# kuldeepbrd1/graspLDM

Measured on AMD Instinct MI355X. Metric: grasps/sec whole-node (1024-pt cloud, 100 DDIM steps), higher is better.
Workload: dtype f32 (GEMMs as split-f16 x3 partial products on the f16 matrix pipe, f32 accumulation; GroupNorm / LayerNorm / attention / scheduler in f32); 1 GPU; LDM mode, 256 synthetic 1024-pt clouds per GPU x 20 grasps, 100 DDIM steps: BASELINE.json configs[2] per GPU (configs[3] = this per-GPU workload on 8 GPUs); experiment=fpc, clouds_per_gpu=256, grasps_per_cloud=20, points=1024, ddim_steps=100, encoder=PVCNNEncoder (shipped fpc config), parallelism=cloud-sharded x1, weights=synthetic recipe seed 0, streams=3

## Files before the change

graspldm_amd/csrc/voxel_conv.hip:

```cpp
#include <hip/hip_runtime.h>
#include <stdint.h>
#include <stdio.h>
#include <stdlib.h>

#include "gldm.h"
#include "wstream.h"
#include "devstate.h"

#define GLDM_API extern "C" __attribute__((visibility("default")))

namespace {

using f32x4 = __attribute__((ext_vector_type(4))) float;
typedef __attribute__((address_space(3))) float lds_f;

#ifdef GLDM_DEBUG_KNOBS
__device__ long long g_c3_stamp[32];
#define GLDM_C3_STAMP(i) \
  do { if (blockIdx.x == 5 && blockIdx.y == (gridDim.y >> 1) && threadIdx.x == 0) g_c3_stamp[i] = (long long)__builtin_readcyclecounter(); } while (0)
#else
#define GLDM_C3_STAMP(i) do {} while (0)
#endif

template <int CTRL>
// ... 194 lines not shown
  float *s_part = lds;
#pragma unroll
  for (int mi = 0; mi < MT; ++mi) {
#pragma unroll
    for (int q = 0; q < 4; ++q) {
      const int co = 16 * mi + 4 * kq + q;
      float s = 0.f, s2 = 0.f;
#pragma unroll
      for (int ni = 0; ni < NTW; ++ni) {
        const float v = acc[mi][ni][q];
        s += v;
        s2 += v * v;
      }
      s = row16_sum(s);
      s2 = row16_sum(s2);
      if (col == 0 && co < cout) {
        s_part[(wave * MT * 16 + co) * 2] = s;
        s_part[(wave * MT * 16 + co) * 2 + 1] = s2;
      }
    }
  }
  GLDM_C3_STAMP(24);
  __syncthreads();
  GLDM_C3_STAMP(25);
  if (tid < cout) {
    float s = 0.f, s2 = 0.f;
    for (int w = 0; w < 4; ++w) {
      s += s_part[(w * MT * 16 + tid) * 2];
      s2 += s_part[(w * MT * 16 + tid) * 2 + 1];
    }
    float *p = partial + (((size_t)b * gridDim.x + blockIdx.x) * cout_total + co0 + tid) * 2;
    p[0] = s;
    p[1] = s2;
  }
  GLDM_C3_STAMP(26);
  if (out_cl) {
#pragma unroll
    for (int ni = 0; ni < NTW; ++ni)
#pragma unroll
      for (int mi = 0; mi < MT; ++mi)
        if (16 * mi + 4 * kq < cout) *reinterpret_cast<f32x4 *>(y + (size_t)gvox[ni] * cout_total + 16 * mi + 4 * kq) = acc[mi][ni];
  } else {
#pragma unroll
    for (int mi = 0; mi < MT; ++mi)
#pragma unroll
      for (int q = 0; q < 4; ++q) {
        const int co = 16 * mi + 4 * kq + q;
        if (co < cout) {
#pragma unroll
          for (int ni = 0; ni < NTW; ++ni) y[(size_t)co * r3 + gvox[ni]] = acc[mi][ni][q];
        }
      }
  }
  GLDM_C3_STAMP(21);
}

typedef __attribute__((ext_vector_type(8))) _Float16 c3_f16x8;
typedef __attribute__((ext_vector_type(2))) _Float16 c3_f16x2;
typedef __attribute__((ext_vector_type(2))) float c3_f32x2;
typedef __attribute__((ext_vector_type(4))) unsigned c3_u32x4;
constexpr int kC3Split = 2;

__device__ __forceinline__ void c3_split(const float (&x)[8], c3_u32x4 (&pl)[kC3Split]) {
#pragma unroll
  for (int q = 0; q < 4; ++q) {
    const float a = x[2 * q], b = x[2 * q + 1];
    const c3_f16x2 h = __builtin_convertvector(c3_f32x2{a, b}, c3_f16x2);
    const float ra = __builtin_fmaf((float)h[0], -1.0f, a), rb = __builtin_fmaf((float)h[1], -1.0f, b);
    pl[0][q] = __builtin_bit_cast(unsigned, h);
    pl[1][q] = __builtin_bit_cast(unsigned, __builtin_convertvector(c3_f32x2{ra, rb}, c3_f16x2));
  }
}
__device__ __forceinline__ f32x4 c3_mfma(const c3_u32x4 &a, const c3_u32x4 &b, const f32x4 &c) {
  return __builtin_amdgcn_mfma_f32_16x16x32_f16(__builtin_bit_cast(c3_f16x8, a), __builtin_bit_cast(c3_f16x8, b), c, 0, 0, 0);
}
__device__ __forceinline__ f32x4 c3_mfma3(const c3_u32x4 (&a)[kC3Split], const c3_u32x4 (&b)[kC3Split], f32x4 acc) {
  acc = c3_mfma(a[0], b[1], acc);
  acc = c3_mfma(a[1], b[0], acc);
  return c3_mfma(a[0], b[0], acc);
}

constexpr int kPairs = 14;

__device__ __forceinline__ float c3_range_pow2(float m) {
  int e = (int)((__float_as_uint(m) >> 23) & 0xffu) - 127;
  if ((e >= -8 && e < 14) || e < -100 || e > 100) return 1.0f;
  e = e < -40 ? -40 : e;
  return __uint_as_float((unsigned)(e - 13 + 127) << 23);
}
__device__ __forceinline__ float c3_pow2_inv(float s) { return __uint_as_float((254u << 23) - __float_as_uint(s)); }
__device__ __forceinline__ float c3_wave_max(float x) {
#pragma unroll
  for (int off = 32; off >= 1; off >>= 1) x = fmaxf(x, __shfl_xor(x, off, 64));
  return x;
}

template <int MT, int R, int ZB, int WAVES, bool ACT = false>
__global__ __launch_bounds__(64 * WAVES, (ZB * 16 / WAVES / 16 >= 6) ? 1 : 2) void conv3d_k3_pl_kernel(const float *__restrict__ x,
                                                                                      const float *__restrict__ wp3,
                                                                                      const float *__restrict__ bias, int cin,
                                                                                      int cout, float *__restrict__ y,
                                                                                      float *__restrict__ partial,
                                                                                      const float *__restrict__ in_coef,
                                                                                      int out_cl) {
  constexpr int r = R, NTW = ZB / WAVES, kThreads = 64 * WAVES, kZParts = R / ZB;
  constexpr int GM = MT % 3 == 0 ? 3 : (MT % 4 == 0 ? 4 : (MT % 2 == 0 ? 2 : 1));
  constexpr int GN = NTW % 3 == 0 ? 3 : (NTW % 2 == 0 ? 2 : 1);
  static_assert(R % ZB == 0 && ZB % WAVES == 0, "whole n-tiles per wave");
  constexpr int MG = MT / GM, NG = NTW / GN;
  constexpr int zp = ZB + 2, nvox = 36 * zp, r3 = r * r * r;
  constexpr int hs = (nvox + 15) & ~15;
  constexpr int kItems = 2 * nvox, kRounds = (kItems + kThreads - 1) / kThreads;
  constexpr bool kDB = R == 24 && ZB == 24;
  constexpr bool kRanged = !ACT;
  extern __shared__ float lds[];
  GLDM_C3_STAMP(0);
  __builtin_amdgcn_s_setprio(3);
  const int tid = threadIdx.x, wave = tid >> 6, lane = tid & 63;
  const int col = lane & 15, kq = lane >> 4;
  const int bpr = r / kBrick;
  const int bxy = blockIdx.x / kZParts, bz0 = (blockIdx.x % kZParts) * ZB;
  const int bx0 = (bxy / bpr) * kBrick, by0 = (bxy % bpr) * kBrick;
  const int b = blockIdx.y;
  const int cblocks = (cin + 15) >> 4, kblocks = kPairs * cblocks;
  x += (size_t)b * cin * r3;
  y += (size_t)b * cout * r3;
  const WStream wv(wp3, lane);
  typedef __attribute__((address_space(3))) c3_u32x4 lds_c4;
  constexpr int kSet = kC3Split * 2 * hs;
  lds_c4 *pl0 = (lds_c4 *)lds;

  int vb[NTW];
#pragma unroll
  for (int ni = 0; ni < NTW; ++ni) {
    const int o = 16 * (wave * NTW + ni) + col;
    const int iz = o % ZB, ixy = o / ZB, ix = ixy >> 2, iy = ixy & 3;
    vb[ni] = (ix * 6 + iy) * zp + iz + (kq & 1) * hs;
  }
  f32x4 acc[MT][NTW];
#pragma unroll
  for (int mi = 0; mi < MT; ++mi) {
    f32x4 bvv;
#pragma unroll
    for (int q = 0; q < 4; ++q) bvv[q] = bias[16 * mi + 4 * kq + q];
#pragma unroll
    for (int ni = 0; ni < NTW; ++ni) acc[mi][ni] = bvv;
  }
  int s_lds[kRounds], s_glb[kRounds];
#pragma unroll
  for (int q = 0; q < kRounds; ++q) {
    const int it = tid + q * kThreads;
    s_lds[q] = -1;
    s_glb[q] = -1;
    if (it < kItems) {
      const int h = it / nvox, v = it - h * nvox;
      const int ixy = v / zp, izp = v - ixy * zp;
      const int gx = bx0 + ixy / 6 - 1, gy = by0 + ixy % 6 - 1, gz = bz0 + izp - 1;
      s_lds[q] = h * hs + v;
      if ((unsigned)gx < (unsigned)r && (unsigned)gy < (unsigned)r && (unsigned)gz < (unsigned)r)
        s_glb[q] = (gx * r + gy) * r + gz + 8 * h * r3;
    }
  }
  {
    const c3_u32x4 z4 = c3_u32x4{0u, 0u, 0u, 0u};
#pragma unroll
    for (int q = 0; q < kRounds; ++q)
      if (s_lds[q] >= 0 && s_glb[q] < 0) {
#pragma unroll
        for (int p3 = 0; p3 < kC3Split; ++p3) {
          pl0[p3 * 2 * hs + s_lds[q]] = z4;
          if constexpr (kDB) pl0[kSet + p3 * 2 * hs + s_lds[q]] = z4;
        }
      }
  }
  float stg[kRounds][8];
  auto stage_load = [&](int cb) {
    const float *xc = x + (size_t)(cb * 16) * r3;
#pragma unroll
    for (int q = 0; q < kRounds; ++q) {
      const int g0 = s_glb[q] >= 0 ? s_glb[q] : 0;
#pragma unroll
      for (int j = 0; j < 8; ++j) stg[q][j] = xc[(size_t)j * r3 + g0];
    }
  };
  float *s_coef = lds + (kDB ? 2 : 1) * kSet * 4;
  if constexpr (ACT) {
    for (int i = tid; i < 2 * cin; i += kThreads) s_coef[i] = in_coef[(size_t)b * cin * 2 + i];
  }
  unsigned s_run_u = 0x3f800000u;
  float *rng = s_coef;
  auto stage_store = [&](int cb) {
    lds_c4 *pl = pl0 + (kDB ? (cb & 1) * kSet : 0);
#pragma unroll
    for (int q = 0; q < kRounds; ++q)
      if (s_glb[q] >= 0) {
        if constexpr (kRanged) {
          const float inv_run = __uint_as_float((254u << 23) - s_run_u);
#pragma unroll
          for (int j = 0; j < 8; ++j) stg[q][j] *= inv_run;
        }
        if constexpr (ACT) {
          const int h = (tid + q * kThreads) / nvox;
          const f32x4 *cf = reinterpret_cast<const f32x4 *>(s_coef + 2 * (16 * cb + 8 * h));
#pragma unroll
          for (int j2 = 0; j2 < 4; ++j2) {
            const f32x4 c4 = cf[j2];
            const float t0 = fmaf(stg[q][2 * j2], c4[0], c4[1]), t1 = fmaf(stg[q][2 * j2 + 1], c4[2], c4[3]);
            stg[q][2 * j2] = t0 * __builtin_amdgcn_rcpf(1.0f + __builtin_amdgcn_exp2f(-1.44269504088896340736f * t0));
            stg[q][2 * j2 + 1] = t1 * __builtin_amdgcn_rcpf(1.0f + __builtin_amdgcn_exp2f(-1.44269504088896340736f * t1));
          }
        }
        c3_u32x4 p3[kC3Split];
        c3_split(stg[q], p3);
#pragma unroll
        for (int k = 0; k < kC3Split; ++k) pl[k * 2 * hs + s_lds[q]] = p3[k];
      }
  };
  GLDM_C3_STAMP(1);
  stage_load(0);
  GLDM_C3_STAMP(2);
  for (int cb = 0; cb < cblocks; ++cb) {
    if constexpr (kRanged) {
      float mx = 0.f;
#pragma unroll
      for (int q = 0; q < kRounds; ++q)
        if (s_glb[q] >= 0) {
#pragma unroll
          for (int j = 0; j < 8; ++j) mx = fmaxf(mx, fabsf(stg[q][j]));
        }
      mx = c3_wave_max(mx);
      if (lane == 0) rng[wave] = mx;
    }
    if (!kDB || kRanged || cb == 0) __syncthreads();
    if constexpr (kRanged) {
      float mx = 0.f;
#pragma unroll
      for (int w8 = 0; w8 < WAVES; ++w8) mx = fmaxf(mx, rng[w8]);
      const unsigned need = __builtin_amdgcn_readfirstlane(__float_as_uint(c3_range_pow2(mx)));
      const unsigned s_new = (cb == 0 || need > s_run_u) ? need : s_run_u;
      if (s_new != s_run_u) {
        const float f = __uint_as_float(s_run_u) * c3_pow2_inv(__uint_as_float(s_new));
#pragma unroll
        for (int mi = 0; mi < MT; ++mi)
#pragma unroll
          for (int ni = 0; ni < NTW; ++ni) acc[mi][ni] *= f;
        s_run_u = s_new;
      }
    }
    if (cb < 3) GLDM_C3_STAMP(3 + 4 * cb);
    stage_store(cb);
    if (cb + 1 < cblocks) stage_load(cb + 1);
    __builtin_amdgcn_sched_barrier(0);
    if (cb < 3) GLDM_C3_STAMP(4 + 4 * cb);
    __syncthreads();
    if (cb < 3) GLDM_C3_STAMP(5 + 4 * cb);
    const lds_c4 *pl = pl0 + (kDB ? (cb & 1) * kSet : 0);
    c3_u32x4 a[2][GM][kC3Split];
    auto load_a = [&](int buf, int step) {
      const int p = step / MG, mg = step - p * MG;
#pragma unroll
      for (int mi = 0; mi < GM; ++mi)
#pragma unroll
        for (int k = 0; k < kC3Split; ++k)
          a[buf][mi][k] = wv.raw_at((((GM * mg + mi) * kblocks + cb * kPairs + p) * kC3Split) * 1024, k * 1024);
    };
    load_a(0, 0);
    __builtin_amdgcn_s_setprio(0);
    constexpr int kSteps = kPairs * MG;
    constexpr int kUnits = kPairs * NG;
    constexpr bool kBPre = NG > 1;
    c3_u32x4 bs[kBPre ? 2 : 1][GN][kC3Split];
    auto load_b = [&](int buf, int unit) {
      const int p = unit / NG, ng = unit - p * NG;
      const int ta = 2 * p, tb = 2 * p + 1 < 27 ? 2 * p + 1 : 26;
      const int offa = ((ta / 9) * 6 + (ta / 3) % 3) * zp + ta % 3, offb = ((tb / 9) * 6 + (tb / 3) % 3) * zp + tb % 3;
      const int toff = (kq >> 1) ? offb : offa;
#pragma unroll
      for (int q = 0; q < GN; ++q)
#pragma unroll
        for (int k = 0; k < kC3Split; ++k) bs[buf][q][k] = pl[k * 2 * hs + vb[GN * ng + q] + toff];
    };
    if (kBPre) load_b(0, 0);
    for (int p0 = 0; p0 < kPairs; p0 += 2) {
#pragma unroll
      for (int pu = 0; pu < 2; ++pu) {
        const int p = p0 + pu;
#pragma unroll
        for (int ng = 0; ng < NG; ++ng) {
          const int unit = p * NG + ng;
          const int bcur = kBPre ? ((pu * NG + ng) & 1) : 0;
          if (kBPre) load_b(bcur ^ 1, unit + 1 < kUnits ? unit + 1 : unit);
          else load_b(0, unit);
#pragma unroll
          for (int mg = 0; mg < MG; ++mg) {
            const int step = p * MG + mg;
            const int cur = (pu * MG + mg) & 1;
            if (ng == 0) load_a(cur ^ 1, step + 1 < kSteps ? step + 1 : step);
            __builtin_amdgcn_sched_barrier(0);
#pragma unroll
            for (int mi = 0; mi < GM; ++mi)
#pragma unroll
              for (int q = 0; q < GN; ++q)
                acc[GM * mg + mi][GN * ng + q] = c3_mfma3(a[cur][mi], bs[bcur][q], acc[GM * mg + mi][GN * ng + q]);
            __builtin_amdgcn_sched_barrier(0);
          }
        }
      }
    }
    if (cb < 3) GLDM_C3_STAMP(6 + 4 * cb);
    __builtin_amdgcn_s_setprio(3);
  }
  __syncthreads();
  GLDM_C3_STAMP(20);
  if constexpr (kRanged) {
    if (s_run_u != 0x3f800000u) {
      const float s_run = __uint_as_float(s_run_u);
#pragma unroll
      for (int mi = 0; mi < MT; ++mi)
#pragma unroll
        for (int ni = 0; ni < NTW; ++ni) acc[mi][ni] *= s_run;
    }
  }
  float *s_part = lds;
#pragma unroll
  for (int mi = 0; mi < MT; ++mi) {
#pragma unroll
    for (int q = 0; q < 4; ++q) {
      const int co = 16 * mi + 4 * kq + q;
      float s = 0.f, s2 = 0.f;
#pragma unroll
      for (int ni = 0; ni < NTW; ++ni) {
        const float v = acc[mi][ni][q];
        s += v;
        s2 += v * v;
      }
      s = row16_sum(s);
      s2 = row16_sum(s2);
      if (col == 0) {
        s_part[(wave * MT * 16 + co) * 2] = s;
        s_part[(wave * MT * 16 + co) * 2 + 1] = s2;
      }
    }
  }
  __syncthreads();
  if (tid < cout) {
    float s = 0.f, s2 = 0.f;
    for (int w = 0; w < WAVES; ++w) {
      s += s_part[(w * MT * 16 + tid) * 2];
      s2 += s_part[(w * MT * 16 + tid) * 2 + 1];
    }
    float *p = partial + (((size_t)b * (gridDim.x / kZParts) + bxy) * cout + tid) * 2;
    if constexpr (kZParts == 1) {
      p[0] = s;
      p[1] = s2;
    } else {
      atomicAdd(p, s);
      atomicAdd(p + 1, s2);
    }
  }
  int gvox[NTW];
  {
    int lane_o = lane;
    asm volatile("" : "+v"(lane_o));
#pragma unroll
    for (int ni = 0; ni < NTW; ++ni) {
      const int o = 16 * (wave * NTW + ni) + (lane_o & 15);
      const int iz = o % ZB, ixy = o / ZB, ix = ixy >> 2, iy = ixy & 3;
      gvox[ni] = ((bx0 + ix) * r + by0 + iy) * r + bz0 + iz;
    }
  }
  if (out_cl) {
#pragma unroll
    for (int ni = 0; ni < NTW; ++ni)
#pragma unroll
      for (int mi = 0; mi < MT; ++mi)
        *reinterpret_cast<f32x4 *>(y + (size_t)gvox[ni] * cout + 16 * mi + 4 * kq) = acc[mi][ni];
  } else {
#pragma unroll
    for (int mi = 0; mi < MT; ++mi)
#pragma unroll
      for (int q = 0; q < 4; ++q) {
        const int co = 16 * mi + 4 * kq + q;
#pragma unroll
        for (int ni = 0; ni < NTW; ++ni) y[(size_t)co * r3 + gvox[ni]] = acc[mi][ni][q];
      }
  }
  GLDM_C3_STAMP(21);
}

template <int MT, int R, int CIN, int WAVES>
__global__ __launch_bounds__(64 * WAVES, 4) void conv3d_k3_fewch_sp_kernel(const float *__restrict__ x,
                                                                           const float *__restrict__ wp3,
                                                                           const float *__restrict__ bias,
                                                                           float *__restrict__ y,
                                                                           float *__restrict__ partial) {
  constexpr int r = R, NTW = R / WAVES, kThreads = 64 * WAVES, zp = R + 2, nvox = 36 * zp, r3 = r * r * r;
  static_assert(R % WAVES == 0, "whole n-tiles per wave");
  constexpr int K = 27 * CIN, KB = (K + 31) / 32, cout = 16 * MT;
  constexpr int cs = nvox + ((nvox & 31) == 0 ? 8 : 0);
  extern __shared__ float lds[];
  const int tid = threadIdx.x, wave = tid >> 6, lane = tid & 63;
  const int col = lane & 15, g = lane >> 4;
  const int bpr = r / kBrick;
  const int bx0 = (blockIdx.x / bpr) * kBrick, by0 = (blockIdx.x % bpr) * kBrick;
  const int b = blockIdx.y;
  x += (size_t)b * CIN * r3;
  y += (size_t)b * cout * r3;
  float mx = 0.f;
  for (int i = tid; i < CIN * nvox; i += kThreads) {
    const int ci = i / nvox, v = i - ci * nvox;
    const int ixy = v / zp, izp = v - ixy * zp;
    const int gx = bx0 + ixy / 6 - 1, gy = by0 + ixy % 6 - 1, gz = izp - 1;
    float val = 0.f;
    if ((unsigned)gx < (unsigned)r && (unsigned)gy < (unsigned)r && (unsigned)gz < (unsigned)r)
      val = x[(size_t)ci * r3 + (gx * r + gy) * r + gz];
    lds[ci * cs + v] = val;
    mx = fmaxf(mx, fabsf(val));
  }
  float *rng = lds + CIN * cs;
  mx = c3_wave_max(mx);
  if (lane == 0) rng[wave] = mx;
  int vb[NTW], gvox[NTW];
#pragma unroll
  for (int ni = 0; ni < NTW; ++ni) {
    const int o = 16 * (wave * NTW + ni) + col;
    const int iz = o % r, ixy = o / r, ix = ixy >> 2, iy = ixy & 3;
    vb[ni] = (ix * 6 + iy) * zp + iz;
    gvox[ni] = ((bx0 + ix) * r + by0 + iy) * r + iz;
  }
  const WStream wv(wp3, lane);
  const lds_f *l3 = (const lds_f *)lds;
  __syncthreads();
  float s_in;
  {
    float m8 = 0.f;
#pragma unroll
    for (int w8 = 0; w8 < WAVES; ++w8) m8 = fmaxf(m8, rng[w8]);
    s_in = c3_range_pow2(__uint_as_float(__builtin_amdgcn_readfirstlane(__float_as_uint(m8))));
  }
  const float inv_in = c3_pow2_inv(s_in);
  f32x4 acc[MT][NTW];
#pragma unroll
  for (int mi = 0; mi < MT; ++mi) {
    const f32x4 bvv = *reinterpret_cast<const f32x4 *>(bias + 16 * mi + 4 * g) * inv_in;
#pragma unroll
    for (int ni = 0; ni < NTW; ++ni) acc[mi][ni] = bvv;
  }
#pragma unroll
  for (int kb = 0; kb < KB; ++kb) {
    c3_u32x4 a[MT][kC3Split];
#pragma unroll
    for (int mi = 0; mi < MT; ++mi)
#pragma unroll
      for (int pl = 0; pl < kC3Split; ++pl) a[mi][pl] = wv.raw_at(((mi * KB + kb) * kC3Split) * 1024, pl * 1024);
    int off[8];
#pragma unroll
    for (int j = 0; j < 8; ++j) {
      const int k = 32 * kb + 8 * g + j;
      const int tap = k / CIN, ci = k - tap * CIN;
      off[j] = k < K ? ci * cs + ((tap / 9) * 6 + (tap / 3) % 3) * zp + tap % 3 : 0;
    }
    float v[2][8];
#pragma unroll
    for (int j = 0; j < 8; ++j) v[0][j] = l3[vb[0] + off[j]];
#pragma unroll
    for (int ni = 0; ni < NTW; ++ni) {
      if (ni + 1 < NTW) {
#pragma unroll
        for (int j = 0; j < 8; ++j) v[(ni + 1) & 1][j] = l3[vb[ni + 1] + off[j]];
      }
      c3_u32x4 b3[kC3Split];
#pragma unroll
      for (int j = 0; j < 8; ++j) v[ni & 1][j] *= inv_in;
      c3_split(v[ni & 1], b3);
#pragma unroll
      for (int mi = 0; mi < MT; ++mi) acc[mi][ni] = c3_mfma3(a[mi], b3, acc[mi][ni]);
    }
  }
  if (s_in != 1.0f) {
#pragma unroll
    for (int mi = 0; mi < MT; ++mi)
#pragma unroll
      for (int ni = 0; ni < NTW; ++ni) acc[mi][ni] *= s_in;
  }
  __syncthreads();
  float *s_part = lds;
#pragma unroll
  for (int mi = 0; mi < MT; ++mi) {
#pragma unroll
    for (int q = 0; q < 4; ++q) {
      const int co = 16 * mi + 4 * g + q;
      float s = 0.f, s2 = 0.f;
#pragma unroll
      for (int ni = 0; ni < NTW; ++ni) {
        const float v = acc[mi][ni][q];
        s += v;
        s2 += v * v;
      }
      s = row16_sum(s);
      s2 = row16_sum(s2);
      if (col == 0) {
        s_part[(wave * MT * 16 + co) * 2] = s;
        s_part[(wave * MT * 16 + co) * 2 + 1] = s2;
      }
    }
  }
  __syncthreads();
  if (tid < cout) {
    float s = 0.f, s2 = 0.f;
    for (int w = 0; w < WAVES; ++w) {
      s += s_part[(w * MT * 16 + tid) * 2];
      s2 += s_part[(w * MT * 16 + tid) * 2 + 1];
    }
    float *p = partial + (((size_t)b * gridDim.x + blockIdx.x) * cout + tid) * 2;
    p[0] = s;
    p[1] = s2;
  }
#pragma unroll
  for (int mi = 0; mi < MT; ++mi)
#pragma unroll
    for (int q = 0; q < 4; ++q) {
      const int co = 16 * mi + 4 * g + q;
#pragma unroll
      for (int ni = 0; ni < NTW; ++ni) y[(size_t)co * r3 + gvox[ni]] = acc[mi][ni][q];
    }
}

__global__ __launch_bounds__(512) void groupnorm_swish_kernel(float *__restrict__ y, const float *__restrict__ partial,
                                                              const float *__restrict__ gamma,
                                                              const float *__restrict__ beta, int c, int r3,
                                                              int nbricks, int groups, float eps,
                                                              float *__restrict__ chan_sum) {
  __shared__ double s_stat[2];
  __shared__ float s_red[8];
  const int g = blockIdx.x, b = blockIdx.y, cpg = c / groups;
  const int tid = threadIdx.x;
  if (tid < 64) {
    double s = 0.0, s2 = 0.0;
    for (int i = tid; i < nbricks * cpg; i += 64) {
      const int br = i / cpg, ch = g * cpg + i % cpg;
      const float *p = partial + (((size_t)b * nbricks + br) * c + ch) * 2;
      s += (double)p[0];
      s2 += (double)p[1];
    }
    for (int off = 32; off >= 1; off >>= 1) {
      s += __shfl_xor(s, off, 64);
      s2 += __shfl_xor(s2, off, 64);
    }
    if (tid == 0) {
      const double n = (double)cpg * r3, mean = s / n;
      s_stat[0] = mean;
      s_stat[1] = 1.0 / sqrt(fmax(s2 / n - mean * mean, 0.0) + (double)eps);
    }
  }
  __syncthreads();
  const float mean = (float)s_stat[0], rstd = (float)s_stat[1];
  for (int cc = 0; cc < cpg; ++cc) {
    const int ch = g * cpg + cc;
    float *row = y + ((size_t)b * c + ch) * r3;
    const float ga = gamma[ch] * rstd, be = beta[ch] - mean * rstd * gamma[ch];
    float acc = 0.f;
    const int n4 = (r3 & 3) ? 0 : r3 >> 2;
    if (r3 & 3) {
      for (int i = tid; i < r3; i += 512) {
        const float t = row[i] * ga + be;
        const float o = t / (1.0f + __expf(-t));
        acc += o;
        row[i] = o;
      }
    }
    for (int i = tid; i < n4; i += 512) {
      float4 v = reinterpret_cast<float4 *>(row)[i];
      float o[4] = {v.x, v.y, v.z, v.w};
#pragma unroll
      for (int q = 0; q < 4; ++q) {
        const float t = o[q] * ga + be;
        o[q] = t / (1.0f + __expf(-t));
        acc += o[q];
      }
      reinterpret_cast<float4 *>(row)[i] = make_float4(o[0], o[1], o[2], o[3]);
    }
    if (chan_sum) {
      for (int off = 32; off >= 1; off >>= 1) acc += __shfl_xor(acc, off, 64);
      __syncthreads();
      if ((tid & 63) == 0) s_red[tid >> 6] = acc;
      __syncthreads();
      if (tid == 0) {
        float t = 0.f;
        for (int w = 0; w < 8; ++w) t += s_red[w];
        chan_sum[(size_t)b * c + ch] = t;
      }
    }
  }
}

__global__ void se_gate_kernel(const float *__restrict__ chan_sum, const float *__restrict__ w1,
                               const float *__restrict__ w2, int c, int hid, int r3, int use_relu,
// ... 381 lines not shown
}

template <int MT, int NTW>
int launch_conv(const float *x, const float *wp, const float *bias, int b, int cin, int cout, int r, float *y,
                float *partial, hipStream_t s, int out_cl, int cout_total = -1, int co0 = 0) {
  if (cout_total < 0) cout_total = cout;
  return cin <= 4 ? launch_conv_jn<MT, NTW, 1>(x, wp, bias, b, cin, cout, r, y, partial, s, cout_total, co0, out_cl)
                  : launch_conv_jn<MT, NTW, 4>(x, wp, bias, b, cin, cout, r, y, partial, s, cout_total, co0, out_cl);
}

template <int MH, int NTW>
int launch_conv_halves(const float *x, const float *wp, const float *bias, int b, int cin, int cout, int r, float *y,
                       float *partial, hipStream_t s, int out_cl) {
  const size_t kblocks = 27 * (size_t)((cin + 15) >> 4);
  const int half = 16 * MH;
  const int rc = launch_conv<MH, NTW>(x, wp, bias, b, cin, half, r, y, partial, s, out_cl, cout, 0);
  if (rc != GLDM_OK) return rc;
  return launch_conv<MH, NTW>(x, wp + (size_t)MH * kblocks * 256, bias + half, b, cin, cout - half, r, y, partial, s, out_cl, cout, half);
}

static int conv3d_k3_impl(const float *x, const float *w_packed, const float *bias, int b, int cin, int cout, int r,
                          float *y, float *partial, int out_cl, gldm_stream_t stream) {
  if (!x || !w_packed || !bias || !y || !partial || b <= 0 || cin <= 0 || cout <= 0 || r <= 0)
    return GLDM_ERR_INVALID_ARG;
  if (out_cl && cout % 4) return GLDM_ERR_UNSUPPORTED;
  hipStream_t s = reinterpret_cast<hipStream_t>(stream);
  const int mt = (cout + 15) / 16, ntw = r / 4;
  if (r % 4 || (size_t)16 * brick_row_stride(r) * 4 > 160 * 1024) return GLDM_ERR_UNSUPPORTED;

#ifdef GLDM_DEBUG_KNOBS
  struct StampDump {
    hipStream_t s; int cin, cout, r;
    ~StampDump() {
      if (!getenv("GLDM_C3_STAMP")) return;
      long long h[32];
      (void)hipStreamSynchronize(s);
      (void)hipMemcpyFromSymbol(h, HIP_SYMBOL(g_c3_stamp), sizeof(h));
      printf("conv3d %d->%d @%d: setup %lld, stage0 issue %lld", cin, cout, r, h[1] - h[0], h[2] - h[1]);
      for (int cb = 0; cb < (cin + 15) / 16 && cb < 3; ++cb)
        printf(" | cb%d: wait %lld store %lld barrier %lld taps %lld", cb, h[3 + 4 * cb] - (cb ? h[2 + 4 * cb] : h[2]),
               h[4 + 4 * cb] - h[3 + 4 * cb], h[5 + 4 * cb] - h[4 + 4 * cb], h[6 + 4 * cb] - h[5 + 4 * cb]);
      printf(" | epilogue %lld (stats %lld, barrier %lld, partials %lld, stores %lld), total %lld", h[21] - h[20], h[24] - h[20],
             h[25] - h[24], h[26] - h[25], h[21] - h[26], h[21] - h[0]);
      for (int cb = 0; cb < 2; ++cb)
        printf(" | cb%d taps: first %lld, second %lld, 2..13 %lld", cb, h[14 + 3 * cb] - h[5 + 4 * cb],
               h[15 + 3 * cb] - h[14 + 3 * cb], h[16 + 3 * cb] - h[15 + 3 * cb]);
      printf("\n");
    }
  } dump{s, cin, cout, r};
#endif
#define GLDM_CONV_CASE(M, N) \
  if (mt == M && ntw == N) return launch_conv<M, N>(x, w_packed, bias, b, cin, cout, r, y, partial, s, out_cl)
  GLDM_CONV_CASE(3, 6);
  GLDM_CONV_CASE(6, 3);
  GLDM_CONV_CASE(2, 8);
  GLDM_CONV_CASE(4, 4);
  GLDM_CONV_CASE(8, 2);
  GLDM_CONV_CASE(2, 4);
  GLDM_CONV_CASE(4, 2);
  GLDM_CONV_CASE(1, 4);
  GLDM_CONV_CASE(2, 2);
  GLDM_CONV_CASE(4, 1);
  GLDM_CONV_CASE(8, 1);
#undef GLDM_CONV_CASE
  if (mt == 4 && ntw == 8) return launch_conv_halves<2, 8>(x, w_packed, bias, b, cin, cout, r, y, partial, s, out_cl);
  if (mt == 16 && ntw == 2) return launch_conv_halves<8, 2>(x, w_packed, bias, b, cin, cout, r, y, partial, s, out_cl);
  if (mt == 8 && ntw == 4) return launch_conv_halves<4, 4>(x, w_packed, bias, b, cin, cout, r, y, partial, s, out_cl);
  return GLDM_ERR_UNSUPPORTED;
}

GLDM_API int gldm_conv3d_k3(const float *x, const float *w_packed, const float *bias, int b, int cin, int cout, int r,
                            float *y, float *partial, gldm_stream_t stream) {
  return conv3d_k3_impl(x, w_packed, bias, b, cin, cout, r, y, partial, 0, stream);
}

GLDM_API int gldm_conv3d_k3_cl(const float *x, const float *w_packed, const float *bias, int b, int cin, int cout, int r,
                               float *y_cl, float *partial, gldm_stream_t stream) {
  return conv3d_k3_impl(x, w_packed, bias, b, cin, cout, r, y_cl, partial, 1, stream);
}

template <int MT, int R, int ZB, int WAVES, bool ACT>
int launch_conv_pl_act(const float *x, const float *wp3, const float *bias, int b, int cin, int cout, float *y, float *partial,
                       const float *in_coef, int out_cl, hipStream_t s) {
  const size_t lds_bytes = (size_t)(R == 24 && ZB == 24 ? 2 : 1) * kC3Split * 2 * ((36 * (ZB + 2) + 15) & ~15) * 16 +
                           (ACT ? (size_t)2 * cin * sizeof(float) : 64 );
  struct Tag {};
  gldm_dev::allow_dynamic_lds<Tag>(reinterpret_cast<const void *>(&conv3d_k3_pl_kernel<MT, R, ZB, WAVES, ACT>), (int)lds_bytes);
  const int bpr = R / kBrick;
  if (R != ZB) {
    if (hipMemsetAsync(partial, 0, (size_t)b * bpr * bpr * cout * 2 * sizeof(float), s) != hipSuccess) return GLDM_ERR_LAUNCH;
  }
  hipLaunchKernelGGL((conv3d_k3_pl_kernel<MT, R, ZB, WAVES, ACT>), dim3(bpr * bpr * (R / ZB), b), dim3(64 * WAVES), lds_bytes,
                     s, x, wp3, bias, cin, cout, y, partial, in_coef, out_cl);
  return hipGetLastError() == hipSuccess ? GLDM_OK : GLDM_ERR_LAUNCH;
}
template <int MT, int R, int ZB, int WAVES>
int launch_conv_pl(const float *x, const float *wp3, const float *bias, int b, int cin, int cout, float *y, float *partial,
                   const float *in_coef, int out_cl, hipStream_t s) {
  return in_coef ? launch_conv_pl_act<MT, R, ZB, WAVES, true>(x, wp3, bias, b, cin, cout, y, partial, in_coef, out_cl, s)
                 : launch_conv_pl_act<MT, R, ZB, WAVES, false>(x, wp3, bias, b, cin, cout, y, partial, nullptr, out_cl, s);
}

static int conv3d_k3_f16x2_impl(const float *x, const float *in_coef, const float *w_split, const float *bias, int b, int cin,
                                 int cout, int r, float *y, float *partial, int out_cl, gldm_stream_t stream) {
  if (!x || !w_split || !bias || !y || !partial || b <= 0 || cin <= 0 || cout <= 0 || r <= 0) return GLDM_ERR_INVALID_ARG;
  if ((in_coef || out_cl) && cin % 16) return GLDM_ERR_UNSUPPORTED;
  hipStream_t s = reinterpret_cast<hipStream_t>(stream);
  if (cin == 3 && cout == 48 && r == 24) {
    constexpr int kZp = 26, kNvox = 36 * kZp;
    const size_t lds_bytes = (size_t)3 * (kNvox + ((kNvox & 31) == 0 ? 8 : 0)) * sizeof(float) + 64;
    hipLaunchKernelGGL((conv3d_k3_fewch_sp_kernel<3, 24, 3, 8>), dim3(36, b), dim3(512), lds_bytes, s, x, w_split, bias, y, partial);
    return hipGetLastError() == hipSuccess ? GLDM_OK : GLDM_ERR_LAUNCH;
  }
  if (cin % 16) return GLDM_ERR_UNSUPPORTED;
#ifdef GLDM_DEBUG_KNOBS
  struct StampDump {
    hipStream_t s; int cin, cout, r, b;
    ~StampDump() {
      if (!getenv("GLDM_C3_STAMP")) return;
      long long h[32];
      (void)hipStreamSynchronize(s);
      (void)hipMemcpyFromSymbol(h, HIP_SYMBOL(g_c3_stamp), sizeof(h));
      printf("conv3d split %d->%d @%d b=%d: setup %lld, stage0 issue %lld", cin, cout, r, b, h[1] - h[0], h[2] - h[1]);
      for (int cb = 0; cb < cin / 16 && cb < 3; ++cb)
        printf(" | cb%d: wait %lld store %lld barrier %lld taps %lld", cb, h[3 + 4 * cb] - (cb ? h[2 + 4 * cb] : h[2]),
               h[4 + 4 * cb] - h[3 + 4 * cb], h[5 + 4 * cb] - h[4 + 4 * cb], h[6 + 4 * cb] - h[5 + 4 * cb]);
      printf(" | epilogue %lld, total %lld\n", h[21] - h[20], h[21] - h[0]);
    }
  } dump{s, cin, cout, r, b};
#endif
  if (cout == 48 && r == 24) return launch_conv_pl<3, 24, 24, 8>(x, w_split, bias, b, cin, cout, y, partial, in_coef, out_cl, s);
  if (cout == 96 && r == 12) return launch_conv_pl<6, 12, 12, 4>(x, w_split, bias, b, cin, cout, y, partial, in_coef, out_cl, s);
  if (cout == 32 && r == 32) return launch_conv_pl<2, 32, 32, 8>(x, w_split, bias, b, cin, cout, y, partial, in_coef, out_cl, s);
  if (cout == 64 && r == 32) return launch_conv_pl<4, 32, 32, 8>(x, w_split, bias, b, cin, cout, y, partial, in_coef, out_cl, s);
  if (cout == 32 && r == 16) return launch_conv_pl<2, 16, 16, 4>(x, w_split, bias, b, cin, cout, y, partial, in_coef, out_cl, s);
  if (cout == 64 && r == 16) return launch_conv_pl<4, 16, 16, 4>(x, w_split, bias, b, cin, cout, y, partial, in_coef, out_cl, s);
  if (cout == 128 && r == 16) return launch_conv_pl<8, 16, 16, 8>(x, w_split, bias, b, cin, cout, y, partial, in_coef, out_cl, s);
  if (cout == 64 && r == 8) return launch_conv_pl<4, 8, 8, 4>(x, w_split, bias, b, cin, cout, y, partial, in_coef, out_cl, s);
  if (cout == 128 && r == 8) return launch_conv_pl<8, 8, 8, 4>(x, w_split, bias, b, cin, cout, y, partial, in_coef, out_cl, s);
  if (cout == 256 && r == 8) return launch_conv_pl<16, 8, 8, 8>(x, w_split, bias, b, cin, cout, y, partial, in_coef, out_cl, s);
  if (cout == 128 && r == 4) return launch_conv_pl<8, 4, 4, 4>(x, w_split, bias, b, cin, cout, y, partial, in_coef, out_cl, s);
  return GLDM_ERR_UNSUPPORTED;
}

GLDM_API int gldm_conv3d_k3_f16x2(const float *x, const float *w_split, const float *bias, int b, int cin, int cout, int r,
                                   float *y, float *partial, gldm_stream_t stream) {
  return conv3d_k3_f16x2_impl(x, nullptr, w_split, bias, b, cin, cout, r, y, partial, 0, stream);
}

GLDM_API int gldm_conv3d_k3_f16x2_gn(const float *x, const float *in_coef, const float *w_split, const float *bias, int b,
                                      int cin, int cout, int r, float *y, float *partial, int out_channel_last,
                                      gldm_stream_t stream) {
  return conv3d_k3_f16x2_impl(x, in_coef, w_split, bias, b, cin, cout, r, y, partial, out_channel_last ? 1 : 0, stream);
}

GLDM_API int gldm_groupnorm_coef(const float *partial, const float *gamma, const float *beta, int b, int c, int r, int groups,
                                 float eps, float *coef, gldm_stream_t stream) {
  if (!partial || !gamma || !beta || !coef || b <= 0 || c <= 0 || r <= 0 || groups <= 0 || c % groups || c / groups > 64)
    return GLDM_ERR_INVALID_ARG;
  const int nbricks = ((r + kBrick - 1) / kBrick) * ((r + kBrick - 1) / kBrick);
  hipLaunchKernelGGL(groupnorm_coef_kernel, dim3(groups, b), dim3(64), 0, reinterpret_cast<hipStream_t>(stream), partial, gamma,
                     beta, c, r * r * r, nbricks, groups, eps, coef);
  return hipGetLastError() == hipSuccess ? GLDM_OK : GLDM_ERR_LAUNCH;
}

GLDM_API int gldm_gn_swish_chan_sum(const float *y, const float *coef, int b, int c, int r, float *chan_sum,
                                    gldm_stream_t stream) {
// ... 121 lines not shown
```

graspldm_amd/voxel.py:

```python
import torch

from . import _lib as L
from .r1d_pack import mfma_a_fragments

SUPPORTED = {(3, 6), (6, 3), (2, 8), (4, 4), (8, 2), (4, 8), (2, 4), (4, 2), (1, 4), (2, 2), (4, 1), (8, 1),
             (16, 2), (8, 4)}


SPLIT_SHAPES = {(48, 24), (96, 12), (32, 32), (64, 32), (32, 16), (64, 16), (128, 16), (64, 8), (128, 8), (256, 8), (128, 4)}


def conv_supported(cout, r):
    return cout % 16 == 0 and r % 4 == 0 and (cout // 16, r // 4) in SUPPORTED


def pack_conv3d(weight):
    cout, cin = weight.shape[:2]
    cpad = (cin + 15) // 16 * 16
    w = torch.zeros(cout, 27, cpad, dtype=torch.float32)
    w[:, :, :cin] = weight.detach().float().cpu().reshape(cout, cin, 27).permute(0, 2, 1)
    return mfma_a_fragments(w.reshape(cout, 27 * cpad))


def split_conv_supported(cin, cout, r):
    if (cin, cout, r) == (3, 48, 24):
        from .numerics import split_enabled
        return split_enabled()
    if cin % 16 or (cout, r) not in SPLIT_SHAPES:
        return False
    from .numerics import split_enabled
    return split_enabled() or not conv_supported(cout, r)


def pack_conv3d_fewch_f16x2(weight):
    from .r1d_pack import mfma_a_fragments_f16x2
    cout, cin = weight.shape[:2]
    k = 27 * cin
    w = torch.zeros(cout, (k + 31) // 32 * 32, dtype=torch.float32)
    w[:, :k] = weight.detach().float().cpu().reshape(cout, cin, 27).permute(0, 2, 1).reshape(cout, k)
    return mfma_a_fragments_f16x2(w)


def pack_conv3d_f16x2(weight):
    from .r1d_pack import mfma_a_fragments_f16x2
    cout, cin = weight.shape[:2]
    cb = cin // 16
    w = torch.zeros(cout, cb, 14, 2, 16, dtype=torch.float32)
    wt = weight.detach().float().cpu().reshape(cout, cb, 16, 27)
    taps = torch.zeros(cout, cb, 16, 28)
    taps[..., :27] = wt
    w[:] = taps.reshape(cout, cb, 16, 14, 2).permute(0, 1, 3, 4, 2)
    return mfma_a_fragments_f16x2(w.reshape(cout, cb * 14 * 32))


class VoxelBranchPlan:

    def __init__(self, convs, device, r=None):
        from .r1d_pack import SplitRangeError
        self.split = [r is not None and split_conv_supported(c.in_channels, c.out_channels, r) for c in convs]
        self.generic = [r is not None and not conv_supported(c.out_channels, r) for c in convs]
        self.w = []
        for i, c in enumerate(convs):
            if self.split[i]:
                try:
                    self.w.append((pack_conv3d_fewch_f16x2(c.weight) if c.in_channels < 16 else pack_conv3d_f16x2(c.weight)).to(device))
                    continue
                except SplitRangeError:
                    self.split[i] = False
            self.w.append((c.weight.detach().float().contiguous() if self.generic[i] else pack_conv3d(c.weight)).to(device))
        self.key = None


def run(plan, convs, norms, se, vox, norm_coords, point_feat, r):
    dev = vox.device
    b = vox.shape[0]
    st = L.current_stream(dev)
    x = vox.contiguous()
    coef = None
    chan_sum = None
    x_cl = False
    with torch.cuda.device(dev):
        for i, (conv, gn) in enumerate(zip(convs, norms)):
            cin, cout = conv.in_channels, conv.out_channels
            y = torch.empty((b, cout, r, r, r), dtype=torch.float32, device=dev)
            nf = L.lib().gldm_conv3d_partial_floats(b, cout, r)
            partial = torch.empty(int(nf), dtype=torch.float32, device=dev)
            last = i == len(convs) - 1
            staged = plan.split[i] and cin % 16 == 0
            mfma32 = not plan.split[i] and not plan.generic[i]
            cl = last and (staged or mfma32) and cout % 4 == 0 and cout <= 256 and cout // gn.num_groups <= 64
            if staged and (coef is not None or cl):
                L.call("gldm_conv3d_k3_f16x2_gn", L.ptr(x), L.ptr(coef), L.ptr(plan.w[i]), L.ptr(conv.bias), b, cin, cout, r,
                       L.ptr(y), L.ptr(partial), 1 if cl else 0, st)
            elif cl:
                assert coef is None
                L.call("gldm_conv3d_k3_cl", L.ptr(x), L.ptr(plan.w[i]), L.ptr(conv.bias), b, cin, cout, r, L.ptr(y), L.ptr(partial), st)
            else:
                assert coef is None
                entry = "gldm_conv3d_k3_generic" if plan.generic[i] else ("gldm_conv3d_k3_f16x2" if plan.split[i] else "gldm_conv3d_k3")
                L.call(entry, L.ptr(x), L.ptr(plan.w[i]), L.ptr(conv.bias), b, cin, cout, r, L.ptr(y), L.ptr(partial), st)
            x_cl = cl
            foldable = (last or (plan.split[i + 1] and convs[i + 1].in_channels % 16 == 0 and r >= 16)) \
                and cout // gn.num_groups <= 64
            if foldable:
                coef = torch.empty((b, cout, 2), dtype=torch.float32, device=dev)
                L.call("gldm_groupnorm_coef", L.ptr(partial), L.ptr(gn.weight), L.ptr(gn.bias), b, cout, r, gn.num_groups,
                       float(gn.eps), L.ptr(coef), st)
            else:
                coef = None
                if last and se is not None:
                    chan_sum = torch.empty((b, cout), dtype=torch.float32, device=dev)
                L.call("gldm_groupnorm_swish", L.ptr(y), L.ptr(partial), L.ptr(gn.weight), L.ptr(gn.bias), b, cout, r,
                       gn.num_groups, float(gn.eps), L.ptr(chan_sum) if (last and se is not None) else None, st)
            x = y
        c = x.shape[1]
        gate = None
        if se is not None:
            gate = torch.empty((b, c), dtype=torch.float32, device=dev)
            w1, w2 = se.fc[0].weight, se.fc[2].weight
            if x_cl:
                parts = int(L.lib().gldm_squeeze_parts())
                chan_sum = torch.empty((b, parts, c), dtype=torch.float32, device=dev)
                L.call("gldm_gn_swish_chan_sum_cl", L.ptr(x), L.ptr(coef), b, c, r, L.ptr(chan_sum), st)
                L.call("gldm_se_gate_parts", L.ptr(chan_sum), parts, L.ptr(w1), L.ptr(w2), b, c, w1.shape[0], r,
                       1 if se.use_relu else 0, L.ptr(gate), st)
            else:
                if coef is not None:
                    chan_sum = torch.empty((b, c), dtype=torch.float32, device=dev)
                    L.call("gldm_gn_swish_chan_sum", L.ptr(x), L.ptr(coef), b, c, r, L.ptr(chan_sum), st)
                L.call("gldm_se_gate", L.ptr(chan_sum), L.ptr(w1), L.ptr(w2), b, c, w1.shape[0], r,
                       1 if se.use_relu else 0, L.ptr(gate), st)
        n = norm_coords.shape[2]
        out = torch.empty((b, c, n), dtype=torch.float32, device=dev)
        pf = point_feat.contiguous() if point_feat is not None else None
        if x_cl:
            L.call("gldm_devoxelize_gn_cl_fused", L.ptr(norm_coords), L.ptr(x), L.ptr(coef), L.ptr(gate), L.ptr(pf), b, c, n, r,
                   L.ptr(out), st)
        elif coef is not None:
            L.call("gldm_devoxelize_gn_fused", L.ptr(norm_coords), L.ptr(x), L.ptr(coef), L.ptr(gate), L.ptr(pf), b, c, n, r,
                   L.ptr(out), st)
        else:
            L.call("gldm_devoxelize_fused", L.ptr(norm_coords), L.ptr(x), L.ptr(gate), L.ptr(pf), b, c, n, r, L.ptr(out), st)
    return out
```

Baseline: 309,500 grasps/s.

## Interleave split planes in LDS, XCD-aware brick order, fold GN at r=12

Adds a C3Planes layout. When ZB is not a multiple of 16, the f16 split planes are interleaved per y-row with a padded row stride, apparently to avoid LDS bank conflicts and cut footprint. Remaps the workgroup index so consecutive bricks of a batch land on the same XCD, for better L2 locality. Also enables folding GroupNorm coefficients into the next conv at resolution 12. This risks layout mistakes in the partial-sum indexing and extra integer math per block.

```diff
diff --git a/graspldm_amd/csrc/voxel_conv.hip b/graspldm_amd/csrc/voxel_conv.hip
--- a/graspldm_amd/csrc/voxel_conv.hip
+++ b/graspldm_amd/csrc/voxel_conv.hip
@@ -300,6 +300,22 @@
 
 constexpr int kPairs = 14;
 
+template <int ZB>
+struct C3Planes {
+  static constexpr int zp = ZB + 2;
+  static constexpr bool kIlv = ZB % 16 != 0;
+  static constexpr int kYS = !kIlv ? zp : kC3Split * zp + ((ZB - kC3Split * zp) % 16 + 16) % 16;
+  static constexpr int kHS = !kIlv ? (36 * zp + 15) & ~15 : 36 * kYS;
+  static constexpr int kPS = !kIlv ? 2 * kHS : zp;
+  static constexpr int kSet = !kIlv ? kC3Split * 2 * kHS : 2 * kHS;
+  static_assert(!kIlv || (kYS % 16 == ZB % 16 && kYS >= kC3Split * zp && kHS % 16 == 0), "plane layout");
+};
+
+__device__ __forceinline__ int xcd_brick_order(int h, int n) {
+  const int q = n >> 3, rem = n & 7, xcd = h & 7;
+  return (xcd < rem ? xcd * (q + 1) : rem + xcd * q) + (h >> 3);
+}
+
 __device__ __forceinline__ float c3_range_pow2(float m) {
   int e = (int)((__float_as_uint(m) >> 23) & 0xffu) - 127;
   if ((e >= -8 && e < 14) || e < -100 || e > 100) return 1.0f;
@@ -327,7 +343,8 @@
   static_assert(R % ZB == 0 && ZB % WAVES == 0, "whole n-tiles per wave");
   constexpr int MG = MT / GM, NG = NTW / GN;
   constexpr int zp = ZB + 2, nvox = 36 * zp, r3 = r * r * r;
-  constexpr int hs = (nvox + 15) & ~15;
+  using PL = C3Planes<ZB>;
+  constexpr int kYS = PL::kYS, kHS = PL::kHS, kPS = PL::kPS;
   constexpr int kItems = 2 * nvox, kRounds = (kItems + kThreads - 1) / kThreads;
   constexpr bool kDB = R == 24 && ZB == 24;
   constexpr bool kRanged = !ACT;
@@ -337,15 +354,16 @@
   const int tid = threadIdx.x, wave = tid >> 6, lane = tid & 63;
   const int col = lane & 15, kq = lane >> 4;
   const int bpr = r / kBrick;
-  const int bxy = blockIdx.x / kZParts, bz0 = (blockIdx.x % kZParts) * ZB;
+  const int wg = xcd_brick_order(blockIdx.y * gridDim.x + blockIdx.x, gridDim.x * gridDim.y);
+  const int blk = wg % gridDim.x, b = wg / gridDim.x;
+  const int bxy = blk / kZParts, bz0 = (blk % kZParts) * ZB;
   const int bx0 = (bxy / bpr) * kBrick, by0 = (bxy % bpr) * kBrick;
-  const int b = blockIdx.y;
   const int cblocks = (cin + 15) >> 4, kblocks = kPairs * cblocks;
   x += (size_t)b * cin * r3;
   y += (size_t)b * cout * r3;
   const WStream wv(wp3, lane);
   typedef __attribute__((address_space(3))) c3_u32x4 lds_c4;
-  constexpr int kSet = kC3Split * 2 * hs;
+  constexpr int kSet = PL::kSet;
   lds_c4 *pl0 = (lds_c4 *)lds;
 
   int vb[NTW];
@@ -353,7 +371,7 @@
   for (int ni = 0; ni < NTW; ++ni) {
     const int o = 16 * (wave * NTW + ni) + col;
     const int iz = o % ZB, ixy = o / ZB, ix = ixy >> 2, iy = ixy & 3;
-    vb[ni] = (ix * 6 + iy) * zp + iz + (kq & 1) * hs;
+    vb[ni] = (ix * 6 + iy) * kYS + iz + (kq & 1) * kHS;
   }
   f32x4 acc[MT][NTW];
 #pragma unroll
@@ -374,7 +392,7 @@
       const int h = it / nvox, v = it - h * nvox;
       const int ixy = v / zp, izp = v - ixy * zp;
       const int gx = bx0 + ixy / 6 - 1, gy = by0 + ixy % 6 - 1, gz = bz0 + izp - 1;
-      s_lds[q] = h * hs + v;
+      s_lds[q] = h * kHS + ixy * kYS + izp;
       if ((unsigned)gx < (unsigned)r && (unsigned)gy < (unsigned)r && (unsigned)gz < (unsigned)r)
         s_glb[q] = (gx * r + gy) * r + gz + 8 * h * r3;
     }
@@ -386,8 +404,8 @@
       if (s_lds[q] >= 0 && s_glb[q] < 0) {
 #pragma unroll
         for (int p3 = 0; p3 < kC3Split; ++p3) {
-          pl0[p3 * 2 * hs + s_lds[q]] = z4;
-          if constexpr (kDB) pl0[kSet + p3 * 2 * hs + s_lds[q]] = z4;
+          pl0[p3 * kPS + s_lds[q]] = z4;
+          if constexpr (kDB) pl0[kSet + p3 * kPS + s_lds[q]] = z4;
         }
       }
   }
@@ -431,7 +449,7 @@
         c3_u32x4 p3[kC3Split];
         c3_split(stg[q], p3);
 #pragma unroll
-        for (int k = 0; k < kC3Split; ++k) pl[k * 2 * hs + s_lds[q]] = p3[k];
+        for (int k = 0; k < kC3Split; ++k) pl[k * kPS + s_lds[q]] = p3[k];
       }
   };
   GLDM_C3_STAMP(1);
@@ -491,12 +509,12 @@
     auto load_b = [&](int buf, int unit) {
       const int p = unit / NG, ng = unit - p * NG;
       const int ta = 2 * p, tb = 2 * p + 1 < 27 ? 2 * p + 1 : 26;
-      const int offa = ((ta / 9) * 6 + (ta / 3) % 3) * zp + ta % 3, offb = ((tb / 9) * 6 + (tb / 3) % 3) * zp + tb % 3;
+      const int offa = ((ta / 9) * 6 + (ta / 3) % 3) * kYS + ta % 3, offb = ((tb / 9) * 6 + (tb / 3) % 3) * kYS + tb % 3;
       const int toff = (kq >> 1) ? offb : offa;
 #pragma unroll
       for (int q = 0; q < GN; ++q)
 #pragma unroll
-        for (int k = 0; k < kC3Split; ++k) bs[buf][q][k] = pl[k * 2 * hs + vb[GN * ng + q] + toff];
+        for (int k = 0; k < kC3Split; ++k) bs[buf][q][k] = pl[k * kPS + vb[GN * ng + q] + toff];
     };
     if (kBPre) load_b(0, 0);
     for (int p0 = 0; p0 < kPairs; p0 += 2) {
@@ -620,8 +638,9 @@
   const int tid = threadIdx.x, wave = tid >> 6, lane = tid & 63;
   const int col = lane & 15, g = lane >> 4;
   const int bpr = r / kBrick;
-  const int bx0 = (blockIdx.x / bpr) * kBrick, by0 = (blockIdx.x % bpr) * kBrick;
-  const int b = blockIdx.y;
+  const int wg = xcd_brick_order(blockIdx.y * gridDim.x + blockIdx.x, gridDim.x * gridDim.y);
+  const int blk = wg % gridDim.x, b = wg / gridDim.x;
+  const int bx0 = (blk / bpr) * kBrick, by0 = (blk % bpr) * kBrick;
   x += (size_t)b * CIN * r3;
   y += (size_t)b * cout * r3;
   float mx = 0.f;
@@ -730,7 +749,7 @@
       s += s_part[(w * MT * 16 + tid) * 2];
       s2 += s_part[(w * MT * 16 + tid) * 2 + 1];
     }
-    float *p = partial + (((size_t)b * gridDim.x + blockIdx.x) * cout + tid) * 2;
+    float *p = partial + (((size_t)b * gridDim.x + blk) * cout + tid) * 2;
     p[0] = s;
     p[1] = s2;
   }
@@ -1278,7 +1297,7 @@
 template <int MT, int R, int ZB, int WAVES, bool ACT>
 int launch_conv_pl_act(const float *x, const float *wp3, const float *bias, int b, int cin, int cout, float *y, float *partial,
                        const float *in_coef, int out_cl, hipStream_t s) {
-  const size_t lds_bytes = (size_t)(R == 24 && ZB == 24 ? 2 : 1) * kC3Split * 2 * ((36 * (ZB + 2) + 15) & ~15) * 16 +
+  const size_t lds_bytes = (size_t)(R == 24 && ZB == 24 ? 2 : 1) * C3Planes<ZB>::kSet * 16 +
                            (ACT ? (size_t)2 * cin * sizeof(float) : 64 );
   struct Tag {};
   gldm_dev::allow_dynamic_lds<Tag>(reinterpret_cast<const void *>(&conv3d_k3_pl_kernel<MT, R, ZB, WAVES, ACT>), (int)lds_bytes);
diff --git a/graspldm_amd/voxel.py b/graspldm_amd/voxel.py
--- a/graspldm_amd/voxel.py
+++ b/graspldm_amd/voxel.py
@@ -100,7 +100,7 @@
                 entry = "gldm_conv3d_k3_generic" if plan.generic[i] else ("gldm_conv3d_k3_f16x2" if plan.split[i] else "gldm_conv3d_k3")
                 L.call(entry, L.ptr(x), L.ptr(plan.w[i]), L.ptr(conv.bias), b, cin, cout, r, L.ptr(y), L.ptr(partial), st)
             x_cl = cl
-            foldable = (last or (plan.split[i + 1] and convs[i + 1].in_channels % 16 == 0 and r >= 16)) \
+            foldable = (last or (plan.split[i + 1] and convs[i + 1].in_channels % 16 == 0 and r >= 12)) \
                 and cout // gn.num_groups <= 64
             if foldable:
                 coef = torch.empty((b, cout, 2), dtype=torch.float32, device=dev)
```

Result: no change. 312,600 grasps/s, median of 6 (+1.0%).
